# myrrix/myrrix-recommender

Measured on AMD Instinct MI355X. Metric: ALS rows solved/sec (full iteration) at k=64, higher is better.
Workload: dtype f32 storage; per-row Gramian: f16x2-split operands (22 bits), f32 accumulate; Cholesky f32

## Files before the change

### myrrix-recommender_amd/csrc/als_kernels.h

```cpp
#pragma once
#include <hip/hip_runtime.h>
#include <stdint.h>

#include <type_traits>

#include "work_plan.h"

namespace mals {

#ifndef MALS_WAVES
#define MALS_WAVES(T, MODE) ((T) <= 4 ? 4 : ((T) == 5 ? 3 : 2))
#endif
#ifndef MALS_WAVES_H
#define MALS_WAVES_H(T, MODE) ((T) <= 2 ? 5 : ((T) <= 4 ? 3 : 2))
#endif

typedef float f32x4 __attribute__((ext_vector_type(4)));
typedef double f64x4 __attribute__((ext_vector_type(4)));

__host__ __device__ constexpr int tri(int T) { return T * (T + 1) / 2; }
__host__ __device__ constexpr int tidx(int T, int i, int j) { return i * T - (i * (i - 1)) / 2 + (j - i); }

constexpr int GRAMIAN_FLUSH_BINADES = 5;
constexpr int YMAX_SLOTS = 64;
// ... 971 lines not shown
    } else {
#pragma unroll
      for (int t = 0; t < tri(T); ++t) acc[t] = f32x4{0.f, 0.f, 0.f, 0.f};
    }
    float bpart[T];
#pragma unroll
    for (int v = 0; v < T; ++v) bpart[v] = 0.f;
#ifdef MALS_PROFILING
    const int64_t trow = it / n_waves - p.trace_start;
    const bool tr = MODE == 0 && p.trace && wave < 64 && trow >= 0 && trow < 64;
    unsigned long long t0 = 0, t1 = 0, t2 = 0, t3 = 0;
    if (tr) t0 = __builtin_readcyclecounter();
    if (!(p.flags & 0x200)) gather_row<T, D, FULL>(p, cur.begin, cur.len, lane, pp, acc, bpart);
    if (tr) t1 = __builtin_readcyclecounter();
#else
    gather_row<T, D, FULL>(p, cur.begin, cur.len, lane, pp, acc, bpart);
#endif
    float bcol[T];
#pragma unroll
    for (int v = 0; v < T; ++v) bcol[v] = reduce_groups(bpart[v], lane);
    const bool prime_next = nxt.len > 0;
    if (prime_next) pp.ch = chunk_issue(p, nxt.begin, nxt.len, 0, lane);
    const WorkItem nxt2 = load_item(p, it + 2 * n_waves);
    if (MODE == 0) {
      const float wmax = p.refine_flag ? fmaxf(row_part_max<T>(acc, sG, lane), p.gramian_weight * __int_as_float(max_entry_bits<T>(acc, lane))) : 0.f;
      add_ridge<T, FULL>(p, acc, cur.len, lane);
      float minpiv = 3.0e38f;
      float xcol[T];
#ifdef MALS_PROFILING
      if (p.flags & 0x100) {
#pragma unroll
        for (int v = 0; v < T; ++v) xcol[v] = 1e-3f + 1e-9f * (bcol[v] + acc[tidx(T, v, v)][0] + acc[tidx(T, 0, v)][1]);
        if (prime_next) {
          chunk_weights(p, pp.ch);
          prime_row<T, D, FULL>(p, lane, pp);
        }
      } else
#endif
      {
        cholesky_tiles<T>(acc, lane, minpiv);
#ifdef MALS_PROFILING
        if (tr) t2 = __builtin_readcyclecounter();
#endif
        if (prime_next) {
          chunk_weights(p, pp.ch);
          prime_row<T, D, FULL>(p, lane, pp);
        }
        solve_tiles<T>(acc, bcol, xcol, lane);
      }
      store_row<T>(p, xcol, minpiv, wmax, cur.id, lane);
#ifdef MALS_PROFILING
      if (tr) {
        t3 = __builtin_readcyclecounter();
        if (lane == 0) {
          unsigned long long* o = p.trace + (trow * 64 + wave) * 6;
          o[0] = t0; o[1] = t1; o[2] = t2; o[3] = t3; o[4] = (unsigned long long)cur.len; o[5] = wall_clock64();
        }
      }
#endif
    } else {
      float* s = p.scratch + (int64_t)cur.id * ((tri(T) * 4 + T) * 64);
#pragma unroll
      for (int t = 0; t < tri(T); ++t) reinterpret_cast<f32x4*>(s)[t * 64 + lane] = acc[t];
#pragma unroll
      for (int v = 0; v < T; ++v) s[(tri(T) * 4 + v) * 64 + lane] = bcol[v];
      if (prime_next) {
        chunk_weights(p, pp.ch);
        prime_row<T, D, FULL>(p, lane, pp);
      }
    }
    if (nxt.len < 0) break;
    cur = nxt;
    nxt = nxt2;
    it += n_waves;
  }
}

template <int T, int MODE, bool FULL, int NTERM = 2>
__global__ __launch_bounds__(256, MALS_WAVES_H(T, MODE)) void als_persistent_kernel_h(SolveParams p) {
  __shared__ f32x4 sG[MODE == 0 ? tri(T) * 64 : 1];
  const int lane = threadIdx.x & 63;
  const int wave = uniform(blockIdx.x * 4 + (threadIdx.x >> 6));
  const int64_t n_waves = (int64_t)gridDim.x * 4;
  if (MODE == 0) {
    const f32x4* G4 = reinterpret_cast<const f32x4*>(p.Gf);
    for (int e = threadIdx.x; e < tri(T) * 64; e += 256) sG[e] = (p.flags & 2) ? f32x4{0.f, 0.f, 0.f, 0.f} : G4[e];
    __syncthreads();
  }
  int64_t it = wave;
  if (it >= p.n_work) return;
  if (p.zscale[2] == 0.f) return;
  const float zscale = __int_as_float(uniform(__float_as_int(p.zscale[0])));
  const float inv_s2 = __int_as_float(uniform(__float_as_int(p.zscale[1])));
  WorkItem cur = load_item(p, it);
  WorkItem nxt = load_item(p, it + n_waves);
  WorkItem nx2 = load_item(p, it + 2 * n_waves);
  constexpr int E = split_slots(T);
  float raw[T][E];
#pragma unroll
  for (int v = 0; v < T; ++v)
#pragma unroll
    for (int e = 0; e < E; ++e) raw[v][e] = 0.f;
  if (cur.len > 0) {
    Chunk ch = chunk_issue<true>(p, cur.begin, cur.len, 0, lane);
    Chunk nch = nxt.len > 0 ? chunk_issue<true>(p, nxt.begin, nxt.len, 0, lane) : ch;
    chunk_weights_h(p, ch, zscale);
    prime_row_h<T, E, FULL>(p, ch.col, lane, raw);
    for (;;) {
      const WorkItem nx3 = load_item(p, it + 3 * n_waves);
      f32x4 acc[tri(T)];
#pragma unroll
      for (int t = 0; t < tri(T); ++t) acc[t] = f32x4{0.f, 0.f, 0.f, 0.f};
      float bpart[T];
#pragma unroll
      for (int v = 0; v < T; ++v) bpart[v] = 0.f;
#ifdef MALS_PROFILING
      const int64_t trow = it / n_waves - p.trace_start;
      const bool tr = MODE == 0 && p.trace && wave < 64 && trow >= 0 && trow < 64;
      unsigned long long t0 = 0, t1 = 0, t2 = 0;
      if (tr) t0 = __builtin_readcyclecounter();
#endif
      gather_row_h<T, E, FULL, NTERM>(p, cur.begin, cur.len, lane, zscale, ch, nch.col, raw, acc, bpart);
#ifdef MALS_PROFILING
      if (tr) t1 = __builtin_readcyclecounter();
#endif
      float bcol[T];
#pragma unroll
      for (int v = 0; v < T; ++v) bcol[v] = reduce_groups(bpart[v], lane);
      ch = nch;
      if (nxt.len > 0) chunk_weights_h(p, ch, zscale);
      if (MODE == 0) {
        const float rmax = p.refine_flag ? __int_as_float(max_entry_bits<T>(acc, lane)) * inv_s2 : 0.f;
#pragma unroll
        for (int t = 0; t < tri(T); ++t) {
          const f32x4 g4 = sG[t * 64 + lane];
          if constexpr (T <= MALS_PK_MAXT) {
            acc[t] = __builtin_elementwise_fma(acc[t], f32x4{inv_s2, inv_s2, inv_s2, inv_s2}, g4);
          } else {
#pragma unroll
            for (int r = 0; r < 4; ++r) acc[t][r] = fmaf(acc[t][r], inv_s2, g4[r]);
          }
        }
        add_ridge<T, FULL>(p, acc, cur.len, lane);
        float minpiv = 3.0e38f, wmax;
        float xcol[T];
        if constexpr (T >= 2) {
          const float inv_s2row = row_scale<T>(acc, bcol, lane, wmax);
          cholesky_tiles<T, true>(acc, lane, minpiv);
          minpiv *= inv_s2row;
        } else {
          wmax = __int_as_float(max_entry_bits<T>(acc, lane));
          cholesky_tiles<T>(acc, lane, minpiv);
        }
#ifdef MALS_PROFILING
        if (tr) t2 = __builtin_readcyclecounter();
#endif
        solve_tiles<T>(acc, bcol, xcol, lane);
        store_row<T>(p, xcol, minpiv, fmaxf(rmax, p.gramian_weight * wmax), cur.id, lane);
#ifdef MALS_PROFILING
        if (tr) {
          const unsigned long long t3 = __builtin_readcyclecounter();
          if (lane == 0) {
            unsigned long long* o = p.trace + (trow * 64 + wave) * 6;
            o[0] = t0; o[1] = t1; o[2] = t2; o[3] = t3; o[4] = (unsigned long long)cur.len; o[5] = wall_clock64();
          }
        }
#endif
      } else {
        float* s = p.scratch + (int64_t)cur.id * ((tri(T) * 4 + T) * 64);
#pragma unroll
        for (int t = 0; t < tri(T); ++t) reinterpret_cast<f32x4*>(s)[t * 64 + lane] = acc[t] * inv_s2;
#pragma unroll
        for (int v = 0; v < T; ++v) s[(tri(T) * 4 + v) * 64 + lane] = bcol[v];
      }
      cur = nxt;
      nxt = nx2;
      nx2 = nx3;
      nch = nxt.len > 0 ? chunk_issue<true>(p, nxt.begin, nxt.len, 0, lane) : nch;
      it += n_waves;
      if (cur.len <= 0) break;
    }
  }
  if (MODE == 0) {
    while (cur.len == 0) {
      f32x4 acc[tri(T)];
#pragma unroll
      for (int t = 0; t < tri(T); ++t) acc[t] = sG[t * 64 + lane];
      float bcol[T];
#pragma unroll
      for (int v = 0; v < T; ++v) bcol[v] = 0.f;
      finish_row<T>(p, acc, bcol, 0, cur.id, lane);
      it += n_waves;
      cur = load_item(p, it);
    }
  }
}

template <int T>
__device__ __forceinline__ void add_slot(const float* __restrict__ s, int lane, f32x4 (&acc)[tri(T)], float (&bcol)[T]) {
  constexpr int PASSES = T >= 6 ? 2 : 1, PER = (tri(T) + PASSES - 1) / PASSES;
#pragma unroll
  for (int ps = 0; ps < PASSES; ++ps) {
    f32x4 part[PER];
#pragma unroll
    for (int t = 0; t < PER; ++t)
      if (ps * PER + t < tri(T)) part[t] = reinterpret_cast<const f32x4*>(s)[(ps * PER + t) * 64 + lane];
    if (ps == 0) {
      float bp[T];
#pragma unroll
      for (int v = 0; v < T; ++v) bp[v] = s[(tri(T) * 4 + v) * 64 + lane];
#pragma unroll
      for (int v = 0; v < T; ++v) bcol[v] += bp[v];
    }
#pragma unroll
    for (int t = 0; t < PER; ++t)
      if (ps * PER + t < tri(T)) acc[ps * PER + t] += part[t];
    if (PASSES > 1) __builtin_amdgcn_sched_barrier(0);
  }
}

template <int T>
__global__ __launch_bounds__(256) void als_prereduce_kernel(SolveParams p) {
  const int lane = threadIdx.x & 63;
  const int64_t wave = (int64_t)blockIdx.x * 4 + (threadIdx.x >> 6);
  if (wave >= p.n_work) return;
  RowC rc = p.rowsC[wave];
  rc.first_slot = uniform64(rc.first_slot);
  rc.nseg = uniform(rc.nseg);
  constexpr int SLOT = (tri(T) * 4 + T) * 64;
  float* s0 = p.scratch + rc.first_slot * (int64_t)SLOT;
  f32x4 acc[tri(T)];
  float bcol[T];
#pragma unroll
  for (int t = 0; t < tri(T); ++t) acc[t] = reinterpret_cast<const f32x4*>(s0)[t * 64 + lane];
#pragma unroll
  for (int v = 0; v < T; ++v) bcol[v] = s0[(tri(T) * 4 + v) * 64 + lane];
  for (int sgi = 1; sgi < rc.nseg; ++sgi) {
    add_slot<T>(s0 + sgi * (int64_t)SLOT, lane, acc, bcol);
  }
#pragma unroll
  for (int t = 0; t < tri(T); ++t) reinterpret_cast<f32x4*>(s0)[t * 64 + lane] = acc[t];
#pragma unroll
  for (int v = 0; v < T; ++v) s0[(tri(T) * 4 + v) * 64 + lane] = bcol[v];
}

template <int T, bool PERM = false>
__global__ __launch_bounds__(256, T >= 6 ? 2 : 1) void als_finish_kernel(SolveParams p) {
  const int lane = threadIdx.x & 63;
  const int64_t wave = (int64_t)blockIdx.x * 4 + (threadIdx.x >> 6);
  if (wave >= p.n_work) return;
  if (PERM && p.zscale[2] == 0.f) return;
  if (!PERM && (p.flags & 8) && p.zscale[2] != 0.f) return;
  RowC rc = p.rowsC[wave];
  rc.first_slot = uniform64(rc.first_slot);
  rc.row = uniform(rc.row);
  rc.nseg = uniform(rc.nseg);
// ... 792 lines not shown
```

### myrrix-recommender_amd/csrc/mals_api.hip

```cpp
#include "../../include/myrrix_als.h"
#include "als_kernels.h"
#include "dual_kernels.h"
#include "lds_kernels.h"
#include "host_eigen.h"
#include "host_solver.h"
#include "mals_internal.h"
#include "mals_handle.h"
#include "hip_buffer.h"
#include "work_plan.h"
#include "convergence.h"

#include <hip/hip_runtime.h>

#include <algorithm>
#include <chrono>
#include <cmath>
#include <cstdio>
#include <cstdlib>
#include <cstring>
#include <limits>
#include <memory>
#include <new>
#include <string>
#include <type_traits>
// ... 77 lines not shown
  HIPCHK(h, d_rows.alloc(rows.size()));
  HIPCHK(h, d_off.alloc(n_off));
  HIPCHK(h, d_unsorted.alloc(rows.size()));
  HIPCHK(h, hipMemcpyAsync(d_rows.get(), rows.data(), sizeof(BandRow) * rows.size(), hipMemcpyHostToDevice, h->stream));
  HIPCHK(h, hipMemsetAsync(d_unsorted.get(), 0, sizeof(int) * rows.size(), h->stream));
  hipLaunchKernelGGL(band_cuts_kernel, dim3((unsigned)rows.size(), BAND_CHECK_SLICES), dim3(256), 0, h->stream, s.col, d_rows.get(),
                     (int)bc.n_bands, bc.band_rows, d_off.get(), d_unsorted.get());
  HIPCHK(h, hipGetLastError());
  bc.off.resize(n_off);
  bc.unsorted.resize(rows.size());
  HIPCHK(h, hipMemcpyAsync(bc.off.data(), d_off.get(), sizeof(int64_t) * n_off, hipMemcpyDeviceToHost, h->stream));
  HIPCHK(h, hipMemcpyAsync(bc.unsorted.data(), d_unsorted.get(), sizeof(int) * rows.size(), hipMemcpyDeviceToHost, h->stream));
  HIPCHK(h, hipStreamSynchronize(h->stream));
  return MALS_OK;
}

int scan_shard(mals_handle h, SideState& s, BandCuts& bc) {
  s.max_abs_val = 0.f;
  s.mean_abs_val = 0.0;
  s.local_mean_abs_val = 0.0;
  if (s.nnz > 0) {
    HIPCHK(h, hipMemsetAsync(h->d_maxabs.get(), 0, 4 * sizeof(unsigned), h->stream));
    const unsigned blocks = (unsigned)std::min<int64_t>(4096, (s.nnz + 255) / 256);
    hipLaunchKernelGGL(max_abs_kernel, dim3(blocks), dim3(256), 0, h->stream, s.val, s.nnz, h->d_maxabs.get(),
                       reinterpret_cast<double*>(h->d_maxabs.get() + 2));
    HIPCHK(h, hipGetLastError());
    unsigned raw[4];
    HIPCHK(h, hipMemcpyAsync(raw, h->d_maxabs.get(), sizeof(raw), hipMemcpyDeviceToHost, h->stream));
    HIPCHK(h, hipStreamSynchronize(h->stream));
    std::memcpy(&s.max_abs_val, &raw[0], sizeof(float));
    double sum = 0.0;
    std::memcpy(&sum, &raw[2], sizeof(double));
    s.mean_abs_val = sum / (double)s.nnz;
    s.local_mean_abs_val = s.mean_abs_val;
  }
  s.local_max_abs_val = s.max_abs_val;
  s.col_min = 0;
  s.col_max = -1;
  if (s.nnz > 0) {
    const int init[2] = {std::numeric_limits<int>::max(), std::numeric_limits<int>::min()};
    HIPCHK(h, hipMemcpyAsync(h->d_colrange.get(), init, sizeof(init), hipMemcpyHostToDevice, h->stream));
    const unsigned blocks = (unsigned)std::min<int64_t>(4096, (s.nnz + 255) / 256);
    hipLaunchKernelGGL(col_range_kernel, dim3(blocks), dim3(256), 0, h->stream, s.col, s.nnz, h->d_colrange.get());
    HIPCHK(h, hipGetLastError());
    int range[2];
    HIPCHK(h, hipMemcpyAsync(range, h->d_colrange.get(), sizeof(range), hipMemcpyDeviceToHost, h->stream));
    HIPCHK(h, hipStreamSynchronize(h->stream));
    s.col_min = range[0];
    s.col_max = range[1];
    if (s.col_min < 0) return fail(h, MALS_INVALID_ARG, "negative column index");
  }
  if (int rc = find_band_cuts(h, s, bc)) return rc;
  {
    const char* e = std::getenv("MALS_BAND_FRONT");
    s.band_front = !e || std::atoi(e) != 0;
  }
  return MALS_OK;
}

int upload_work_lists(mals_handle h, SideState& s, const WorkPlan& plan, const BandCuts& bc) {
  s.chunks = plan.chunks;
  s.n_dual_rows = plan.n_dual_rows;
  if (std::getenv("MALS_DEBUG_LISTS")) {
    int64_t nd[4] = {0, 0, 0, 0}, ed[4] = {0, 0, 0, 0}, na = 0, nz = 0, n_long = 0;
    for (const ChunkRange& cr : s.chunks) {
      n_long += cr.nC;
      for (int c = 0; c < 4; ++c) {
        nd[c] += cr.nD[c];
        ed[c] += cr.nnzD[c];
      }
      na += cr.nA;
      nz += cr.nZ;
    }
    std::fprintf(stderr, "[lists] rows %lld: direct %lld (%lld entries), dual 1-16: %lld (%lld) 17-32: %lld (%lld) 33-48: %lld (%lld) 49-64: %lld (%lld), "
                         "zero-filled %lld, segments %lld of %lld long rows (%lld entries)\n",
                 (long long)s.n_local, (long long)na, (long long)plan.nnzA, (long long)nd[0], (long long)ed[0], (long long)nd[1], (long long)ed[1], (long long)nd[2],
                 (long long)ed[2], (long long)nd[3], (long long)ed[3], (long long)nz, (long long)plan.itemsB.size(), (long long)n_long, (long long)plan.nnzB);
    int64_t e_band = 0;
    for (const ChunkRange& cr : s.chunks) e_band += cr.nnzBand;
    std::fprintf(stderr, "[lists] bands %lld of %lld table rows (at least %lld entries per band): %lld banded rows (%lld entries) in %lld segments, "
                         "%lld long enough but unsorted\n",
                 (long long)bc.n_bands, (long long)bc.band_rows, (long long)bc.min_avg, (long long)plan.n_banded_rows, (long long)e_band,
                 (long long)plan.n_banded_segs, (long long)plan.n_unsorted);
  }
  if (!plan.itemsA.empty()) {
    HIPCHK(h, s.itemsA.alloc(plan.itemsA.size()));
    HIPCHK(h, hipMemcpy(s.itemsA.get(), plan.itemsA.data(), sizeof(WorkItem) * plan.itemsA.size(), hipMemcpyHostToDevice));
  }
  if (!plan.itemsB.empty()) {
    HIPCHK(h, s.itemsB.alloc(plan.itemsB.size()));
    HIPCHK(h, hipMemcpy(s.itemsB.get(), plan.itemsB.data(), sizeof(WorkItem) * plan.itemsB.size(), hipMemcpyHostToDevice));
    HIPCHK(h, s.rowsC.alloc(plan.rowsC.size()));
    HIPCHK(h, hipMemcpy(s.rowsC.get(), plan.rowsC.data(), sizeof(RowC) * plan.rowsC.size(), hipMemcpyHostToDevice));
    HIPCHK(h, s.scratch.alloc((size_t)(plan.n_slots * slot_floats(h->T))));
  }
  return MALS_OK;
}

int64_t wanted_chunk_rows(mals_handle h, const SideState& s) { return s.chunk_rows_override >= 0 ? s.chunk_rows_override : h->cfg.chunk_rows; }

int build_work_lists(mals_handle h, SideState& s) {
  BandCuts bc;
  WorkPlan plan;
  s.n_dual_rows = 0;
  if (int rc = scan_shard(h, s, bc)) return rc;
  if (const char* why = plan_work_lists(s.h_row_ptr.data(), s.n_local, h->cfg.segment_nnz, wanted_chunk_rows(h, s), h->dual_blocks, h->n_cu, bc, plan))
    return fail(h, MALS_INVALID_ARG, why);
  return upload_work_lists(h, s, plan, bc);
}

int validate_matrix(mals_handle h, int side) {
  SideState& s = h->side[side];
  if (s.h_row_ptr.size() != (size_t)s.n_local + 1 || s.h_row_ptr[0] != 0 || s.h_row_ptr[(size_t)s.n_local] != s.nnz)
    return fail(h, MALS_INVALID_ARG, "row_ptr must have n_rows_local+1 entries, start at 0 and end at nnz");
  return MALS_OK;
}

int validate_columns(mals_handle h, int side) {
  const SideState& s = h->side[side];
  const SideState& o = h->side[1 - side];
  if (s.nnz > 0 && o.n_total > 0 && (int64_t)s.col_max >= o.n_total)
    return fail(h, MALS_INVALID_ARG, "column index outside the opposite side's factor replica");
  return MALS_OK;
}

int begin_timed(mals_handle h, int kind, double bytes, PendingEvent& pe) {
  pe.kind = kind;
  pe.bytes = bytes;
  if (!h->timing) return MALS_OK;
  HIPCHK(h, pe.ev.ensure());
  HIPCHK(h, hipEventRecord(pe.ev.begin, h->stream));
  return MALS_OK;
}
int end_timed(mals_handle h, PendingEvent& pe) {
  if (!h->timing) return MALS_OK;
  HIPCHK(h, hipEventRecord(pe.ev.end, h->stream));
  h->pending.push_back(std::move(pe));
  return MALS_OK;
}
int drain_events(mals_handle h) {
  const std::vector<PendingEvent> pending = std::move(h->pending);
  h->pending.clear();
  for (const PendingEvent& pe : pending) {
    HIPCHK(h, hipEventSynchronize(pe.ev.end));
    float ms = 0.f;
    HIPCHK(h, hipEventElapsedTime(&ms, pe.ev.begin, pe.ev.end));
    mals_stats& st = h->stats;
    switch (pe.kind) {
      case 0: st.rows_ms += ms; st.rows_launches += 1; st.rows_bytes += pe.bytes; break;
      case 1: st.segments_ms += ms; st.segments_launches += 1; st.segments_bytes += pe.bytes; break;
      case 2: st.finish_ms += ms; st.finish_launches += 1; st.finish_bytes += pe.bytes; break;
      case 4: st.dual_ms += ms; st.dual_launches += 1; st.dual_bytes += pe.bytes; break;
      case 5: st.rotate_ms += ms; st.rotate_launches += 1; st.rotate_bytes += pe.bytes; break;
      default: st.gramian_ms += ms; st.gramian_launches += 1; st.gramian_bytes += pe.bytes; break;
    }
  }
  return MALS_OK;
}

template <int MIN_T = 1, typename F>
int dispatch_T(mals_handle h, F&& f) {
  if (h->T == MIN_T) return f(std::integral_constant<int, MIN_T>());
  if constexpr (MIN_T < 8) return dispatch_T<MIN_T + 1>(h, f);
  return fail(h, MALS_INVALID_ARG, "unsupported feature count");
}
constexpr int gather_depth(int T) { return T <= 3 ? 4 : T == 4 ? MALS_D4 : 2; }

constexpr int64_t GRAMIAN_SPLIT_MIN_ROWS = 262144;
inline int64_t gramian_slab_rows(int64_t n_rows) {
  static const int64_t forced = std::getenv("MALS_GRAMIAN_SLAB_ROWS") ? std::atoll(std::getenv("MALS_GRAMIAN_SLAB_ROWS")) : 0;
  if (forced > 0) return forced;
  int64_t slab = 512;
  while (slab < 2048 && n_rows / (2 * slab) / 4 >= 1024) slab *= 2;
  return slab;
}

template <int T>
int launch_gramian_T(mals_handle h, SideState& s, const float* M, int64_t n_rows, double* G_out, float* Gf_out, unsigned* ymax) {
  const int k = h->cfg.features;
  const int elems = tri(T) * 256;
  static const bool force_f64 = std::getenv("MALS_GRAMIAN_F64") != nullptr;
  if (n_rows >= GRAMIAN_SPLIT_MIN_ROWS && !force_f64) {
    const int64_t slab_rows = gramian_slab_rows(n_rows);
    int64_t n_slabs = (n_rows + slab_rows - 1) / slab_rows;
    n_slabs = (n_slabs + 3) & ~(int64_t)3;
    constexpr int GROUPS = 64;
    const size_t slab_bytes = sizeof(float) * (size_t)n_slabs * tri(T) * 256;
    const size_t bytes = 2 * slab_bytes + sizeof(double) * (size_t)GROUPS * tri(T) * 256 + sizeof(int) * (size_t)n_slabs;
    if (s.partials.capacity() < bytes) HIPCHK(h, s.partials.alloc(bytes));
// ... 21 lines not shown
  if (ymax) HIPCHK(h, hipMemsetAsync(ymax, 0x7f, sizeof(unsigned), h->stream));
  hipLaunchKernelGGL((gramian_partial_kernel<T>), dim3((unsigned)(n_waves / 4)), dim3(256), 0, h->stream, M, n_rows, k,
                     rows_per_wave, partials);
  hipLaunchKernelGGL((gramian_finalize_kernel<T, true, 16>), dim3(elems / 16), dim3(256), 0, h->stream, partials, n_waves,
                     k, G_out, Gf_out);
  HIPCHK(h, hipGetLastError());
  return MALS_OK;
}

int launch_gramian(mals_handle h, SideState& s, const float* M, int64_t n_rows, double* G_out, float* Gf_out, unsigned* ymax = nullptr) {
  return dispatch_T(h, [&](auto t) { return launch_gramian_T<t()>(h, s, M, n_rows, G_out, Gf_out, ymax); });
}

template <typename K>
int persistent_grid(mals_handle h, K kernel, int64_t n_work, unsigned* grid, bool front = false, int block = 256, int resident_per_cu = 0) {
  const int64_t groups = (n_work + block / 64 - 1) / (block / 64);
  if (front) {
    *grid = (unsigned)std::max<int64_t>(1, groups);
    return MALS_OK;
  }
  int per_cu = resident_per_cu;
  if (!per_cu) HIPCHK(h, hipOccupancyMaxActiveBlocksPerMultiprocessor(&per_cu, kernel, 256, 0));
  if (per_cu < 1) per_cu = 1;
  per_cu *= 16;
  if (const char* e = std::getenv("MALS_BLOCKS_PER_CU")) per_cu = std::max(1, std::atoi(e)) * (256 / block);
  const int64_t cap = (int64_t)h->n_cu * per_cu;
  *grid = (unsigned)std::max<int64_t>(1, std::min<int64_t>(groups, cap));
  return MALS_OK;
}

enum { LISTS_ROWS = 1, LISTS_DUAL_ROWS = 2, LISTS_LONG = 4 };

template <typename KR, typename KS, typename KRF, typename KSF, typename KC, typename KCF, typename KP>
struct ListKernels {
  KR rows;
  KS segments;
  KRF rows_f32;
  KSF segments_f32;
  KC finish;
  KCF finish_f32;
  KP prereduce;
  int block;
  int resident_per_cu;
};
template <typename KR, typename KS, typename KRF, typename KSF, typename KC, typename KCF, typename KP>
ListKernels(KR, KS, KRF, KSF, KC, KCF, KP, int, int) -> ListKernels<KR, KS, KRF, KSF, KC, KCF, KP>;

template <typename K, typename KF>
int launch_persistent(mals_handle h, K kernel, KF fallback, int block, int resident_per_cu, const SolveParams& p, int kind, double bytes, bool front) {
  PendingEvent pe;
  unsigned grid = 1;
  if (int rc = persistent_grid(h, kernel, p.n_work, &grid, front, block, resident_per_cu)) return rc;
  if (int rc = begin_timed(h, kind, bytes, pe)) return rc;
  hipLaunchKernelGGL(kernel, dim3(grid), dim3(block), 0, h->stream, p);
  if constexpr (!std::is_same<KF, std::nullptr_t>::value) {
    SolveParams pf = p;
    pf.flags |= 8;
    if (int rc = persistent_grid(h, fallback, p.n_work, &grid)) return rc;
    grid = std::min<unsigned>(grid, (unsigned)h->n_cu * 8u);
    hipLaunchKernelGGL(fallback, dim3(grid), dim3(256), 0, h->stream, pf);
  }
  return end_timed(h, pe);
}

template <typename LK>
int launch_lists(mals_handle h, SideState& s, SolveParams p, int chunk, int which, const LK& fam) {
  const double per = 4.0 * p.k + 8.0;
  const ChunkRange& cr = s.chunks[(size_t)chunk];
  const bool own = which & LISTS_ROWS, longs = which & LISTS_LONG, dual_rows_too = which & LISTS_DUAL_ROWS;
  const WorkItem *A = s.itemsA.get() + cr.offA, *B = s.itemsB.get() + cr.offB;
  const int64_t n_plain = cr.nB - cr.nBand, n_dual = cr.n_dual();
  struct Run {
    const WorkItem* items;
    int64_t n;
    double bytes;
    int kind;
    bool front;
  };
  const Run runs[4] = {
      {B, longs ? n_plain : 0, (double)(cr.nnzB - cr.nnzBand) * per, 1, false},
      {B + n_plain, longs ? cr.nBand : 0, (double)cr.nnzBand * per, 1, s.band_front},
      {A, own ? cr.nA : 0, (double)cr.nnzA * per + (double)cr.nA * per, 0, false},
      {A + cr.nA, dual_rows_too ? n_dual : 0, (double)cr.nnz_dual() * per + (double)n_dual * per, 0, false}};
  for (const Run& r : runs) {
    if (!r.n) continue;
    p.n_work = r.n;
    p.items = r.items;
    if (int rc = r.kind ? launch_persistent(h, fam.segments, fam.segments_f32, fam.block, fam.resident_per_cu, p, 1, r.bytes, r.front)
                        : launch_persistent(h, fam.rows, fam.rows_f32, fam.block, fam.resident_per_cu, p, 0, r.bytes, r.front))
      return rc;
  }
  if (longs && cr.nC) {
    PendingEvent pe;
    if (int rc = begin_timed(h, 2, (double)cr.nC * per, pe)) return rc;
    if (cr.nP) {
      p.n_work = cr.nP;
      p.rowsC = s.rowsC.get() + cr.offP;
      hipLaunchKernelGGL(fam.prereduce, dim3((unsigned)((cr.nP + 3) / 4)), dim3(256), 0, h->stream, p);
    }
    p.n_work = cr.nC;
    p.rowsC = s.rowsC.get() + cr.offC;
    hipLaunchKernelGGL(fam.finish, dim3((unsigned)((cr.nC + 3) / 4)), dim3(256), 0, h->stream, p);
    if constexpr (!std::is_same<decltype(fam.finish_f32), std::nullptr_t>::value) {
      SolveParams pf = p;
      pf.flags |= 8;
      hipLaunchKernelGGL(fam.finish_f32, dim3((unsigned)((cr.nC + 3) / 4)), dim3(256), 0, h->stream, pf);
    }
    if (int rc = end_timed(h, pe)) return rc;
  }
  if (own && cr.nZ) {
    hipLaunchKernelGGL(zero_rows_kernel, dim3((unsigned)((cr.nZ + 31) / 32)), dim3(256), 0, h->stream,
                       A + cr.nA + n_dual, cr.nZ, p.k, p.out);
  }
  HIPCHK(h, hipGetLastError());
  return MALS_OK;
}

template <int T, bool FULL>
int launch_solve_TF(mals_handle h, SideState& s, const SolveParams& p, int chunk, int which) {
  constexpr int D = gather_depth(T);
  constexpr auto rows_f32 = als_persistent_kernel<T, D, 0, FULL>;
  constexpr auto segments_f32 = als_persistent_kernel<T, D, 1, FULL>;
  if constexpr (T == 8 && FULL) {
    if (h->split_f16 && h->lds_gather && p.Gperm)
      return launch_lists(h, s, p, chunk, which, ListKernels{als_lds_kernel_h<0>, als_lds_kernel_h<1>, rows_f32, segments_f32, als_finish_kernel<T, true>,
                                                             als_finish_kernel<T, false>, als_prereduce_kernel<T>, 64, 8});
  }
  if constexpr (T == 4) {
    if (h->split3)
      return launch_lists(h, s, p, chunk, which, ListKernels{als_persistent_kernel_h<T, 0, FULL, 3>, als_persistent_kernel_h<T, 1, FULL, 3>, rows_f32,
                                                             segments_f32, als_finish_kernel<T>, nullptr, als_prereduce_kernel<T>, 256, 0});
  }
  if (h->split_f16)
    return launch_lists(h, s, p, chunk, which, ListKernels{als_persistent_kernel_h<T, 0, FULL>, als_persistent_kernel_h<T, 1, FULL>, rows_f32,
                                                           segments_f32, als_finish_kernel<T>, nullptr, als_prereduce_kernel<T>, 256, 0});
  return launch_lists(h, s, p, chunk, which,
                      ListKernels{rows_f32, segments_f32, nullptr, nullptr, als_finish_kernel<T>, nullptr, als_prereduce_kernel<T>, 256, 0});
}

int launch_solve(mals_handle h, SideState& s, const SolveParams& p, int chunk, int which) {
  return dispatch_T(h, [&](auto t) {
    return p.k == 16 * t() ? launch_solve_TF<t(), true>(h, s, p, chunk, which) : launch_solve_TF<t(), false>(h, s, p, chunk, which);
  });
}

int launch_refine(mals_handle h, const RefineParams& q) {
  const int64_t rows = q.row_end - q.row_begin;
  const unsigned grid = (unsigned)std::max<int64_t>(1, std::min<int64_t>((rows + 255) / 256, (int64_t)h->n_cu * 8));
  return dispatch_T(h, [&](auto t) -> int {
    hipLaunchKernelGGL((als_refine_kernel<t()>), dim3(grid), dim3(256), 0, h->stream, q);
    HIPCHK(h, hipGetLastError());
    return MALS_OK;
  });
}

int launch_gramian_ref(mals_handle h, const SideState& o) {
  const unsigned grid = (unsigned)std::max<int64_t>(1, std::min<int64_t>((o.n_total + 63) / 64, (int64_t)h->n_cu * 2));
  return dispatch_T(h, [&](auto t) -> int {
    hipLaunchKernelGGL(gramian_ref_latch_kernel, dim3(1), dim3(1), 0, h->stream, h->d_gref_state.get());
    hipLaunchKernelGGL((gramian_ref_kernel<t()>), dim3(grid), dim3(256), 0, h->stream, o.F, o.n_total, h->cfg.features, h->d_gref_state.get(),
                       h->d_gref_part.get(), h->d_Gref.get());
    HIPCHK(h, hipGetLastError());
    return MALS_OK;
  });
}

int launch_exact(mals_handle h, const RefineParams& q, int level) {
  const int k = h->cfg.features;
  const size_t lds = sizeof(double) * ((size_t)k * (k + 1) + 2 * (size_t)k) + sizeof(float) * (size_t)k + sizeof(int) * 256;
  if (!h->exact_ready) {
// ... 376 lines not shown
  std::unique_ptr<mals_handle_s> owner(new (std::nothrow) mals_handle_s());
  const mals_handle h = owner.get();
  if (!h) return create_fail(MALS_OOM, "mals_create: out of host memory");
  h->cfg = *cfg;
  h->cfg.flags &= 3;
#ifdef MALS_PROFILING
  if (const char* dbg = std::getenv("MALS_DEBUG_FLAGS")) h->cfg.flags |= (std::atoi(dbg) & 0xff) << 8;
#endif
  if (h->cfg.segment_nnz <= 0) h->cfg.segment_nnz = 4096;
  if (h->cfg.chunk_rows < 0) h->cfg.chunk_rows = 0;
  h->cfg.segment_nnz = (h->cfg.segment_nnz + 3) & ~3;
  h->T = (cfg->features + 15) / 16;
  switch (cfg->gramian_mode) {
    case MALS_GRAMIAN_AUTO: h->split_f16 = h->T >= 2; break;
    case MALS_GRAMIAN_FP32: h->split_f16 = false; break;
    case MALS_GRAMIAN_SPLIT_F16: h->split_f16 = true; break;
    case MALS_GRAMIAN_SPLIT3_F16:
      if (h->T != 4) return create_fail(MALS_INVALID_ARG, "mals_create: MALS_GRAMIAN_SPLIT3_F16 is built for 49..64 features");
      h->split_f16 = h->split3 = true;
      break;
    default: return create_fail(MALS_INVALID_ARG, "mals_create: unknown gramian_mode");
  }
  if (cfg->alpha < 0.0) h->split_f16 = false;
  switch (cfg->solve_mode) {
    case MALS_SOLVE_AUTO: h->dual_blocks = h->T >= 3 ? dual_max_blocks(h->T) : 0; break;
    case MALS_SOLVE_DIRECT: h->dual_blocks = 0; break;
    case MALS_SOLVE_DUAL: h->dual_blocks = dual_max_blocks(h->T); break;
    default: return create_fail(MALS_INVALID_ARG, "mals_create: unknown solve_mode");
  }
  if (h->cfg.flags != 0 || !(cfg->alpha > 0.0)) h->dual_blocks = 0;
  {
    hipDeviceProp_t prop;
    if (hipGetDeviceProperties(&prop, cfg->device) == hipSuccess && prop.multiProcessorCount > 0)
      h->n_cu = prop.multiProcessorCount;
  }
  std::memset(&h->stats, 0, sizeof(h->stats));
  h->stats.struct_size = (int32_t)sizeof(mals_stats);
  hipError_t st = hipSetDevice(cfg->device);
  if (st == hipSuccess) st = h->d_bad.alloc(4);
  if (st == hipSuccess) st = h->h_bad.alloc(4);
  if (st == hipSuccess) st = h->d_zscale.alloc(4);
  if (st == hipSuccess) st = h->d_maxabs.alloc(4);
  if (st == hipSuccess) st = h->d_colrange.alloc(2);
  if (st == hipSuccess) st = h->d_refined.alloc(1);
  if (st == hipSuccess) st = h->d_gref_state.alloc(4);
  if (st == hipSuccess) st = hipMemset(h->d_gref_state.get(), 0, 4 * sizeof(int));
  if (st == hipSuccess) st = hipMemset(h->d_refined.get(), 0, sizeof(unsigned long long));
  if (st == hipSuccess) st = hipMemset(h->d_zscale.get(), 0, 4 * sizeof(float));
  if (st == hipSuccess) st = hipMemset(h->d_bad.get(), 0xff, 4 * sizeof(unsigned long long));
  if (st != hipSuccess) return create_fail(MALS_HIP_ERROR, "mals_create: device " + std::to_string(cfg->device) + ": " + hipGetErrorString(st));
  if (const char* e = std::getenv("MALS_REFINE_LIMIT")) h->refine_limit = std::max(0.f, (float)std::atof(e));
  if (h->ev_ready.ensure(hipEventDisableTiming) != hipSuccess || h->ev_refine.ensure(hipEventDisableTiming) != hipSuccess)
    return create_fail(MALS_HIP_ERROR, "mals_create: creating the handle's events failed");
  h->lds_gather = h->cfg.features == 128;
  if (const char* e = std::getenv("MALS_LDS_GATHER")) h->lds_gather = h->lds_gather && std::atoi(e) != 0;
  if (const char* e = std::getenv("MALS_OVERLAP")) h->overlap = std::atoi(e) != 0;
  if (h->overlap) {
    bool ok = h->ev_fork.ensure(hipEventDisableTiming) == hipSuccess;
    for (int i = 0; i < 2 && ok; ++i) ok = h->aux[i].ensure() == hipSuccess && h->ev_join[i].ensure(hipEventDisableTiming) == hipSuccess;
    if (!ok) h->overlap = false;
  }
#ifdef MALS_PROFILING
  if (std::getenv("MALS_DEBUG_TRACE")) {
    (void)h->d_trace.alloc(64 * 64 * 6);
    (void)hipMemset(h->d_trace.get(), 0, 64 * 64 * 6 * sizeof(unsigned long long));
  }
#endif
  t_create_error.clear();
  malsi_serving_create(h);
  *out = owner.release();
  return MALS_OK;
}

int mals_destroy(mals_handle h) {
  if (!h) return MALS_INVALID_ARG;
  (void)hipSetDevice(h->cfg.device);
  malsi_serving_stop_front(h);
  (void)hipStreamSynchronize(h->stream);
  for (const Stream& a : h->aux)
    if (a) (void)hipStreamSynchronize(a);
  if (h->d_trace) {
    std::vector<unsigned long long> t(64 * 64 * 6);
    (void)hipMemcpy(t.data(), h->d_trace.get(), t.size() * sizeof(unsigned long long), hipMemcpyDeviceToHost);
    for (int r = 0; r < 64; r += 21)
      for (int w = 0; w < 4; w += 1) {
        const unsigned long long* o = &t[(size_t)(r * 64 + w) * 6];
        std::fprintf(stderr, "[trace] iter %2d wave %2d len %5llu gather %7llu chol %7llu solve+store %7llu gap_to_prev_end %lld\n", r, w, o[4],
                     o[1] - o[0], o[2] - o[1], o[3] - o[2], r ? (long long)(o[0] - t[(size_t)((r - 1) * 64 + w) * 6 + 3]) : 0ll);
      }
    for (int w = 0; w < 4; ++w) {
      const unsigned long long* a = &t[(size_t)w * 6];
      const unsigned long long* b = &t[(size_t)(63 * 64 + w) * 6];
      if (b[5] > a[5]) std::fprintf(stderr, "[trace] wave %d: %llu cycles in %llu wall ticks (100 MHz) = %.0f MHz; %.0f cycles per row\n", w, b[3] - a[3], b[5] - a[5], 100.0 * (double)(b[3] - a[3]) / (double)(b[5] - a[5]), (double)(b[3] - a[3]) / 63.0);
    }
  }
  malsi_serving_free(h);
  delete h;
  return MALS_OK;
}

int mals_features(mals_handle h) { return h ? h->cfg.features : 0; }

const char* mals_last_error(mals_handle h) { return h ? h->err.c_str() : "null handle"; }

int mals_set_stream(mals_handle h, void* hip_stream) {
  if (!h) return MALS_INVALID_ARG;
  h->stream = (hipStream_t)hip_stream;
  return MALS_OK;
}

int mals_set_factor_rows(mals_handle h, int side, int64_t n_rows_total) {
  CHECK_SIDE(h, side);
  if (n_rows_total <= 0) return fail(h, MALS_INVALID_ARG, "n_rows_total must be positive");
  if (int rc = use_device(h)) return rc;
  SideState& s = h->side[side];
  s.F = nullptr;
  const size_t n = (size_t)n_rows_total * (size_t)h->cfg.features;
  HIPCHK(h, s.F_own.alloc(n));
  s.F = s.F_own.get();
  HIPCHK(h, hipMemsetAsync(s.F, 0, sizeof(float) * n, h->stream));
  s.n_total = n_rows_total;
  s.G_valid = false;
  ++s.F_epoch;
  if (side == MALS_SIDE_X) h->grown_users_end.store(-1);
  malsi_generation_drop_recent(h, side);
  if (side == MALS_SIDE_X) popular_touch(h, false);
  if (side == MALS_SIDE_Y) h->lsh.clear();
  return MALS_OK;
}

int mals_bind_factors(mals_handle h, int side, float* device_ptr, int64_t n_rows_total) {
  CHECK_SIDE(h, side);
  if (!device_ptr || n_rows_total <= 0) return fail(h, MALS_INVALID_ARG, "null buffer or non-positive row count");
  if (int rc = use_device(h)) return rc;
  SideState& s = h->side[side];
  s.F_own.reset();
  s.F = device_ptr;
  s.n_total = n_rows_total;
  s.G_valid = false;
  ++s.F_epoch;
  if (side == MALS_SIDE_X) h->grown_users_end.store(-1);
  malsi_generation_drop_recent(h, side);
  if (side == MALS_SIDE_X) popular_touch(h, false);
  if (side == MALS_SIDE_Y) h->lsh.clear();
  return MALS_OK;
}

int mals_factor_device_ptr(mals_handle h, int side, void** out_device_ptr, int64_t* out_n_rows_total) {
  CHECK_SIDE(h, side);
  if (out_device_ptr) *out_device_ptr = h->side[side].F;
  if (out_n_rows_total) *out_n_rows_total = h->side[side].n_total;
  return h->side[side].F ? MALS_OK : fail(h, MALS_INVALID_ARG, "factor replica not allocated");
}

int mals_set_matrix(mals_handle h, int side, int64_t row_offset, int64_t n_rows_local, int64_t nnz, const int64_t* row_ptr,
                    const int32_t* col_idx, const float* val, int mem_kind) {
  CHECK_SIDE(h, side);
  if (row_offset < 0 || n_rows_local < 0 || nnz < 0 || !row_ptr || (nnz > 0 && (!col_idx || !val)))
    return fail(h, MALS_INVALID_ARG, "bad matrix arguments");
  if (n_rows_local > std::numeric_limits<int32_t>::max())
    return fail(h, MALS_INVALID_ARG, "at most 2^31-1 local rows per handle");
  if (int rc = use_device(h)) return rc;
  SideState& s = h->side[side];
  HIPCHK(h, hipStreamSynchronize(h->stream));
  free_matrix(s);
  if (side == MALS_SIDE_X) malsi_clear_known_items(h);
  if (side == MALS_SIDE_X) malsi_popular_new_generation(h, true);
// ... 929 lines not shown
```

### myrrix-recommender_amd/csrc/work_plan.h

```cpp
#pragma once

#include "band_plan.h"

#include <algorithm>
#include <cstdint>
#include <limits>
#include <utility>
#include <vector>

namespace mals {

struct WorkItem {
  int64_t begin;
  int32_t len;
  int32_t id;
};
struct RowC {
  int64_t first_slot;
  int32_t row;
  int32_t nseg;
  int32_t stride;
  int32_t pad_;
};
constexpr int FINISH_GROUP = 32;

struct BandCuts {
  int64_t n_bands = 1, band_rows = 0, min_avg = 0;
  std::vector<int64_t> row;
  std::vector<int64_t> off;
  std::vector<int> unsorted;
};

struct ChunkRange {
  int64_t row0 = 0, row1 = 0;
  int64_t offA = 0, nA = 0, nnzA = 0, offB = 0, nB = 0, nnzB = 0, offC = 0, nC = 0;
  int64_t offP = 0, nP = 0;
  int64_t nD[4] = {0, 0, 0, 0}, nnzD[4] = {0, 0, 0, 0}, nZ = 0;
  int64_t nBand = 0, nnzBand = 0;
  int64_t n_dual() const { return nD[0] + nD[1] + nD[2] + nD[3]; }
  int64_t nnz_dual() const { return nnzD[0] + nnzD[1] + nnzD[2] + nnzD[3]; }
};

struct WorkPlan {
  std::vector<WorkItem> itemsA;
  std::vector<WorkItem> itemsB;
  std::vector<RowC> rowsC;
  std::vector<ChunkRange> chunks;
  int64_t n_slots = 0;
  int64_t nnzA = 0, nnzB = 0;
  int64_t n_dual_rows = 0;
  int64_t n_banded_rows = 0, n_banded_segs = 0, n_unsorted = 0;
};

inline int64_t plan_chunk_rows(int64_t chunk_rows, int64_t n_local) { return chunk_rows > 0 ? chunk_rows : std::max<int64_t>(n_local, 1); }

inline const char* plan_work_lists(const int64_t* rp, int64_t n, int seg, int64_t chunk_rows_wanted, int dual_blocks, int n_cu,
                                   const BandCuts& bc, WorkPlan& plan) {
  plan = WorkPlan();
  const int64_t chunk_rows = plan_chunk_rows(chunk_rows_wanted, n);
  const int n_chunks = (int)std::max<int64_t>(1, (n + chunk_rows - 1) / chunk_rows);
  std::vector<WorkItem>& order = plan.itemsA;
  std::vector<WorkItem>& segs = plan.itemsB;
  std::vector<RowC>& rowsC = plan.rowsC;
  std::vector<std::pair<int32_t, WorkItem>> band_segs;
  std::vector<BandPiece> pieces;
  std::vector<RowC> groups;
  size_t bc_next = 0;
  order.reserve((size_t)n);
  int64_t& slot = plan.n_slots;
  plan.chunks.assign((size_t)n_chunks, ChunkRange());
  std::vector<int64_t> count((size_t)seg + 2);
  for (int c = 0; c < n_chunks; ++c) {
    ChunkRange& cr = plan.chunks[(size_t)c];
    const int64_t r0 = cr.row0 = std::min(n, c * chunk_rows), r1 = cr.row1 = std::min(n, (c + 1) * chunk_rows);
    cr.offA = (int64_t)order.size();
    cr.offB = (int64_t)segs.size();
    cr.offC = (int64_t)rowsC.size();
    std::fill(count.begin(), count.end(), 0);
    const int64_t dual_len = 16 * (int64_t)dual_blocks;
    int64_t n_short = 0, n_direct = 0, n_empty = 0;
    for (int64_t r = r0; r < r1; ++r) {
      const int64_t len = rp[r + 1] - rp[r];
      if (len < 0) return "row_ptr must be non-decreasing";
      if (len <= seg) {
        ++count[(size_t)(seg - len)];
        ++n_short;
        if (len == 0) {
          ++n_empty;
        } else if (len <= dual_len) {
          const int cls = (int)((len - 1) >> 4);
          ++cr.nD[cls];
          cr.nnzD[cls] += len;
        } else {
          ++n_direct;
          cr.nnzA += len;
        }
      } else {
        cr.nnzB += len;
      }
    }
    int64_t seg_b = seg;
    {
      const int64_t want_segments = (int64_t)n_cu * 4;
      const int64_t lo = std::min<int64_t>(512, seg);
      seg_b = std::max<int64_t>(lo, std::min<int64_t>(seg, (cr.nnzB + want_segments - 1) / want_segments));
      seg_b = (seg_b + 31) & ~(int64_t)31;
      if (seg_b > seg) seg_b = seg;
    }
    int64_t acc = cr.offA;
    for (size_t b = 0; b < count.size(); ++b) {
      const int64_t cnt = count[b];
      count[b] = acc;
      acc += cnt;
    }
    order.resize((size_t)(cr.offA + n_short));
    for (int64_t r = r0; r < r1; ++r) {
      const int64_t len = rp[r + 1] - rp[r];
      if (len <= seg) {
        WorkItem& w = order[(size_t)count[(size_t)(seg - len)]++];
        w.begin = rp[r];
        w.len = (int32_t)len;
        w.id = (int32_t)r;
      } else {
        const int64_t nseg = (len + seg_b - 1) / seg_b;
        int64_t per = (len + nseg - 1) / nseg;
        per = (per + 3) & ~(int64_t)3;
        RowC rc;
        rc.first_slot = slot;
        rc.row = (int32_t)r;
        rc.nseg = 0;
        rc.stride = 1;
        rc.pad_ = 0;
        pieces.clear();
        if (bc_next < bc.row.size() && bc.row[bc_next] == r) {
          if (bc.unsorted[bc_next]) ++plan.n_unsorted;
          else if (!band_plan_row(&bc.off[bc_next * (size_t)(bc.n_bands + 1)], bc.n_bands, len, seg, pieces)) pieces.clear();
          ++bc_next;
        }
        if (!pieces.empty()) {
          ++plan.n_banded_rows;
          plan.n_banded_segs += (int64_t)pieces.size();
          cr.nnzBand += len;
          for (const BandPiece& pc : pieces) {
            if (slot >= std::numeric_limits<int32_t>::max()) return "too many row segments";
            WorkItem sg;
            sg.begin = rp[r] + pc.begin;
            sg.len = pc.len;
            sg.id = (int32_t)slot++;
            band_segs.emplace_back(pc.band, sg);
            ++rc.nseg;
          }
        } else {
          for (int64_t b = 0; b < len; b += per) {
            if (slot >= std::numeric_limits<int32_t>::max()) return "too many row segments";
            WorkItem sg;
            sg.begin = rp[r] + b;
            sg.len = (int32_t)std::min(per, len - b);
            sg.id = (int32_t)slot++;
            segs.push_back(sg);
            ++rc.nseg;
          }
        }
        if (rc.nseg > FINISH_GROUP) {
          const int32_t grp_len = FINISH_GROUP;
          for (int32_t g0 = 0; g0 < rc.nseg; g0 += grp_len) {
            RowC grp;
            grp.first_slot = rc.first_slot + g0;
            grp.row = (int32_t)r;
            grp.nseg = std::min<int32_t>(grp_len, rc.nseg - g0);
            grp.stride = 1;
            grp.pad_ = 0;
            groups.push_back(grp);
          }
          rc.nseg = (rc.nseg + grp_len - 1) / grp_len;
          rc.stride = grp_len;
        }
        rowsC.push_back(rc);
      }
    }
    const int64_t n_dual = cr.n_dual();
    if (n_empty > 0 && n_dual > 0) {
      auto first = order.begin() + (size_t)(cr.offA + n_direct);
      std::rotate(first, first + (size_t)n_dual, first + (size_t)n_dual + 1);
    }
    cr.nA = n_direct + (n_empty > 0 ? 1 : 0);
    cr.nZ = n_empty > 0 ? n_empty - 1 : 0;
    plan.n_dual_rows += n_dual;
    cr.nBand = (int64_t)band_segs.size();
    cr.nB = (int64_t)segs.size() - cr.offB + cr.nBand;
    cr.nC = (int64_t)rowsC.size() - cr.offC;
    cr.offP = (int64_t)rowsC.size();
    cr.nP = (int64_t)groups.size();
    rowsC.insert(rowsC.end(), groups.begin(), groups.end());
    groups.clear();
    std::stable_sort(segs.begin() + cr.offB, segs.end(), [](const WorkItem& a, const WorkItem& b) { return a.len > b.len; });
    std::stable_sort(band_segs.begin(), band_segs.end(), [](const std::pair<int32_t, WorkItem>& a, const std::pair<int32_t, WorkItem>& b) {
      return a.first != b.first ? a.first < b.first : a.second.len > b.second.len;
    });
    for (const std::pair<int32_t, WorkItem>& bs : band_segs) segs.push_back(bs.second);
    band_segs.clear();
    plan.nnzA += cr.nnzA;
    plan.nnzB += cr.nnzB;
  }
  return nullptr;
}

}
```

Before: 138.7 million.

## Merge consecutive long-row segments into capped runs to cut partial-slot overhead

Long rows split into segments now have adjacent segments (same band) merged into longer work items, capped by a per-launch entry budget derived from wave count and segment size. This reduces the number of partial Gramian slots written to scratch and later reduced, cutting per-item fixed overhead such as the scratch store and finish work. It risks load imbalance when merged items become long relative to the launch. Profiling hooks for segment launches and extra plan statistics are also added under debug flags.

```diff
diff --git a/myrrix-recommender_amd/csrc/als_kernels.h b/myrrix-recommender_amd/csrc/als_kernels.h
--- a/myrrix-recommender_amd/csrc/als_kernels.h
+++ b/myrrix-recommender_amd/csrc/als_kernels.h
@@ -1077,6 +1077,9 @@
   const int lane = threadIdx.x & 63;
   const int wave = uniform(blockIdx.x * 4 + (threadIdx.x >> 6));
   const int64_t n_waves = (int64_t)gridDim.x * 4;
+#ifdef MALS_PROFILING
+  const unsigned long long t_entry = __builtin_readcyclecounter();
+#endif
   if (MODE == 0) {
     const f32x4* G4 = reinterpret_cast<const f32x4*>(p.Gf);
     for (int e = threadIdx.x; e < tri(T) * 64; e += 256) sG[e] = (p.flags & 2) ? f32x4{0.f, 0.f, 0.f, 0.f} : G4[e];
@@ -1101,6 +1104,9 @@
     Chunk nch = nxt.len > 0 ? chunk_issue<true>(p, nxt.begin, nxt.len, 0, lane) : ch;
     chunk_weights_h(p, ch, zscale);
     prime_row_h<T, E, FULL>(p, ch.col, lane, raw);
+#ifdef MALS_PROFILING
+    unsigned long long t_item = t_entry;
+#endif
     for (;;) {
       const WorkItem nx3 = load_item(p, it + 3 * n_waves);
       f32x4 acc[tri(T)];
@@ -1113,11 +1119,13 @@
       const int64_t trow = it / n_waves - p.trace_start;
       const bool tr = MODE == 0 && p.trace && wave < 64 && trow >= 0 && trow < 64;
       unsigned long long t0 = 0, t1 = 0, t2 = 0;
-      if (tr) t0 = __builtin_readcyclecounter();
+      const int64_t every = p.trace_start > 0 ? p.trace_start : 1;
+      const bool tr1 = MODE == 1 && p.trace && it % every == 0 && it / every < 64 * 64;
+      if (tr || tr1) t0 = __builtin_readcyclecounter();
 #endif
       gather_row_h<T, E, FULL, NTERM>(p, cur.begin, cur.len, lane, zscale, ch, nch.col, raw, acc, bpart);
 #ifdef MALS_PROFILING
-      if (tr) t1 = __builtin_readcyclecounter();
+      if (tr || tr1) t1 = __builtin_readcyclecounter();
 #endif
       float bcol[T];
 #pragma unroll
@@ -1167,6 +1175,14 @@
         for (int t = 0; t < tri(T); ++t) reinterpret_cast<f32x4*>(s)[t * 64 + lane] = acc[t] * inv_s2;
 #pragma unroll
         for (int v = 0; v < T; ++v) s[(tri(T) * 4 + v) * 64 + lane] = bcol[v];
+#ifdef MALS_PROFILING
+        const unsigned long long t3 = __builtin_readcyclecounter();
+        if (tr1 && lane == 0) {
+          unsigned long long* o = p.trace + (it / every) * 6;
+          o[0] = t_item; o[1] = t0; o[2] = t1; o[3] = t3; o[4] = (unsigned long long)cur.len; o[5] = wall_clock64();
+        }
+        t_item = t3;
+#endif
       }
       cur = nxt;
       nxt = nx2;
diff --git a/myrrix-recommender_amd/csrc/mals_api.hip b/myrrix-recommender_amd/csrc/mals_api.hip
--- a/myrrix-recommender_amd/csrc/mals_api.hip
+++ b/myrrix-recommender_amd/csrc/mals_api.hip
@@ -183,6 +183,15 @@
                          "%lld long enough but unsorted\n",
                  (long long)bc.n_bands, (long long)bc.band_rows, (long long)bc.min_avg, (long long)plan.n_banded_rows, (long long)e_band,
                  (long long)plan.n_banded_segs, (long long)plan.n_unsorted);
+    int64_t n_plain = 0, n_band = 0, n_groups = 0;
+    for (const ChunkRange& cr : s.chunks) {
+      n_plain += cr.nB - cr.nBand;
+      n_band += cr.nBand;
+      n_groups += cr.nP;
+    }
+    std::fprintf(stderr, "[lists] runs: %lld segments in %lld items of list B (%lld plain, %lld banded), a partial slot of %lld bytes each; %lld slot groups\n",
+                 (long long)plan.n_segments, (long long)plan.n_slots, (long long)n_plain, (long long)n_band, (long long)(slot_floats(h->T) * 4),
+                 (long long)n_groups);
   }
   if (!plan.itemsA.empty()) {
     HIPCHK(h, s.itemsA.alloc(plan.itemsA.size()));
@@ -200,12 +209,23 @@
 
 int64_t wanted_chunk_rows(mals_handle h, const SideState& s) { return s.chunk_rows_override >= 0 ? s.chunk_rows_override : h->cfg.chunk_rows; }
 
+RunRule run_rule(mals_handle h) {
+  RunRule rule;
+  if (h->T > 4) return rule;
+  const int per_simd = h->split_f16 ? MALS_WAVES_H(h->T, 1) : MALS_WAVES(h->T, 1);
+  rule.waves = (int64_t)h->n_cu * 4 * per_simd;
+  rule.longest = 3 * (int64_t)h->cfg.segment_nnz / 2;
+  if (const char* e = std::getenv("MALS_RUN_ENTRIES")) rule.max_entries = std::max<int64_t>(0, std::atoll(e));
+  return rule;
+}
+
 int build_work_lists(mals_handle h, SideState& s) {
   BandCuts bc;
   WorkPlan plan;
   s.n_dual_rows = 0;
   if (int rc = scan_shard(h, s, bc)) return rc;
-  if (const char* why = plan_work_lists(s.h_row_ptr.data(), s.n_local, h->cfg.segment_nnz, wanted_chunk_rows(h, s), h->dual_blocks, h->n_cu, bc, plan))
+  if (const char* why = plan_work_lists(s.h_row_ptr.data(), s.n_local, h->cfg.segment_nnz, wanted_chunk_rows(h, s), h->dual_blocks, h->n_cu, bc, plan,
+                                        run_rule(h)))
     return fail(h, MALS_INVALID_ARG, why);
   return upload_work_lists(h, s, plan, bc);
 }
@@ -393,10 +413,18 @@
       {B + n_plain, longs ? cr.nBand : 0, (double)cr.nnzBand * per, 1, s.band_front},
       {A, own ? cr.nA : 0, (double)cr.nnzA * per + (double)cr.nA * per, 0, false},
       {A + cr.nA, dual_rows_too ? n_dual : 0, (double)cr.nnz_dual() * per + (double)n_dual * per, 0, false}};
+#ifdef MALS_PROFILING
+  unsigned long long* const trace = p.trace;
+  const char* tl = std::getenv("MALS_DEBUG_TRACE_LAUNCH");
+  const int traced_launch = tl ? std::atoi(tl) : 2;
+#endif
   for (const Run& r : runs) {
     if (!r.n) continue;
     p.n_work = r.n;
     p.items = r.items;
+#ifdef MALS_PROFILING
+    p.trace = &r - runs == traced_launch ? trace : nullptr;
+#endif
     if (int rc = r.kind ? launch_persistent(h, fam.segments, fam.segments_f32, fam.block, fam.resident_per_cu, p, 1, r.bytes, r.front)
                         : launch_persistent(h, fam.rows, fam.rows_f32, fam.block, fam.resident_per_cu, p, 0, r.bytes, r.front))
       return rc;
@@ -939,7 +967,27 @@
   if (h->d_trace) {
     std::vector<unsigned long long> t(64 * 64 * 6);
     (void)hipMemcpy(t.data(), h->d_trace.get(), t.size() * sizeof(unsigned long long), hipMemcpyDeviceToHost);
-    for (int r = 0; r < 64; r += 21)
+    const char* tl = std::getenv("MALS_DEBUG_TRACE_LAUNCH");
+    if (tl && std::atoi(tl) < 2) {
+      unsigned long long n = 0, len = 0, total = 0, gather = 0, head = 0, tail = 0;
+      for (size_t i = 0; i < 64 * 64; ++i) {
+        const unsigned long long* o = &t[i * 6];
+        if (!o[3]) continue;
+        ++n;
+        len += o[4];
+        total += o[3] - o[0];
+        gather += o[2] - o[1];
+        head += o[1] - o[0];
+        tail += o[3] - o[2];
+      }
+      if (n)
+        std::fprintf(stderr, "[trace] segments launch %d: %llu sampled items, mean %.0f entries, %.0f cycles per item: gather %.0f, before it %.0f, after it %.0f "
+                             "(%.1f %% outside the gather)\n",
+                     std::atoi(tl), n, (double)len / n, (double)total / n, (double)gather / n, (double)head / n, (double)tail / n,
+                     100.0 * (double)(total - gather) / (double)total);
+      std::fill(t.begin(), t.end(), 0ull);
+    }
+    for (int r = 0; r < 64 && t[3]; r += 21)
       for (int w = 0; w < 4; w += 1) {
         const unsigned long long* o = &t[(size_t)(r * 64 + w) * 6];
         std::fprintf(stderr, "[trace] iter %2d wave %2d len %5llu gather %7llu chol %7llu solve+store %7llu gap_to_prev_end %lld\n", r, w, o[4],
diff --git a/myrrix-recommender_amd/csrc/work_plan.h b/myrrix-recommender_amd/csrc/work_plan.h
--- a/myrrix-recommender_amd/csrc/work_plan.h
+++ b/myrrix-recommender_amd/csrc/work_plan.h
@@ -23,6 +23,23 @@
   int32_t pad_;
 };
 constexpr int FINISH_GROUP = 32;
+
+struct RunRule {
+  int64_t waves = 0;
+  int64_t longest = 0;
+  int64_t max_entries = -1;
+  int64_t cap(int64_t launch_entries) const {
+    int64_t c = max_entries >= 0 ? max_entries : waves > 0 ? launch_entries / (4 * waves) : 0;
+    if (max_entries < 0 && longest > 0 && c > longest) c = longest;
+    return c < (int64_t(1) << 30) ? c : (int64_t(1) << 30);
+  }
+};
+
+inline void plan_runs(int64_t n, int64_t seg_len, int64_t cap, std::vector<int32_t>& per_run) {
+  const int64_t most = std::max<int64_t>(1, seg_len > 0 ? cap / seg_len : 1);
+  const int64_t n_runs = (n + most - 1) / most;
+  for (int64_t i = 0; i < n_runs; ++i) per_run.push_back((int32_t)(n / n_runs + (i < n % n_runs ? 1 : 0)));
+}
 
 struct BandCuts {
   int64_t n_bands = 1, band_rows = 0, min_avg = 0;
@@ -47,6 +64,7 @@
   std::vector<RowC> rowsC;
   std::vector<ChunkRange> chunks;
   int64_t n_slots = 0;
+  int64_t n_segments = 0;
   int64_t nnzA = 0, nnzB = 0;
   int64_t n_dual_rows = 0;
   int64_t n_banded_rows = 0, n_banded_segs = 0, n_unsorted = 0;
@@ -55,7 +73,7 @@
 inline int64_t plan_chunk_rows(int64_t chunk_rows, int64_t n_local) { return chunk_rows > 0 ? chunk_rows : std::max<int64_t>(n_local, 1); }
 
 inline const char* plan_work_lists(const int64_t* rp, int64_t n, int seg, int64_t chunk_rows_wanted, int dual_blocks, int n_cu,
-                                   const BandCuts& bc, WorkPlan& plan) {
+                                   const BandCuts& bc, WorkPlan& plan, const RunRule& runs = RunRule()) {
   plan = WorkPlan();
   const int64_t chunk_rows = plan_chunk_rows(chunk_rows_wanted, n);
   const int n_chunks = (int)std::max<int64_t>(1, (n + chunk_rows - 1) / chunk_rows);
@@ -64,8 +82,19 @@
   std::vector<RowC>& rowsC = plan.rowsC;
   std::vector<std::pair<int32_t, WorkItem>> band_segs;
   std::vector<BandPiece> pieces;
+  std::vector<int32_t> per_run;
   std::vector<RowC> groups;
   size_t bc_next = 0;
+  auto banded_pieces = [&](int64_t r, int64_t len, size_t& cursor) {
+    bool unsorted = false;
+    pieces.clear();
+    if (cursor < bc.row.size() && bc.row[cursor] == r) {
+      if (bc.unsorted[cursor]) unsorted = true;
+      else if (!band_plan_row(&bc.off[cursor * (size_t)(bc.n_bands + 1)], bc.n_bands, len, seg, pieces)) pieces.clear();
+      ++cursor;
+    }
+    return unsorted;
+  };
   order.reserve((size_t)n);
   int64_t& slot = plan.n_slots;
   plan.chunks.assign((size_t)n_chunks, ChunkRange());
@@ -78,7 +107,9 @@
     cr.offC = (int64_t)rowsC.size();
     std::fill(count.begin(), count.end(), 0);
     const int64_t dual_len = 16 * (int64_t)dual_blocks;
-    int64_t n_short = 0, n_direct = 0, n_empty = 0;
+    int64_t n_short = 0, n_direct = 0, n_empty = 0, nnz_band = 0;
+    const bool cap_from_launch = runs.max_entries < 0 && runs.waves > 0;
+    size_t bc_scan = bc_next;
     for (int64_t r = r0; r < r1; ++r) {
       const int64_t len = rp[r + 1] - rp[r];
       if (len < 0) return "row_ptr must be non-decreasing";
@@ -97,8 +128,13 @@
         }
       } else {
         cr.nnzB += len;
+        if (cap_from_launch) {
+          banded_pieces(r, len, bc_scan);
+          if (!pieces.empty()) nnz_band += len;
+        }
       }
     }
+    const int64_t cap_plain = runs.cap(cr.nnzB - nnz_band), cap_band = runs.cap(nnz_band);
     int64_t seg_b = seg;
     {
       const int64_t want_segments = (int64_t)n_cu * 4;
@@ -131,34 +167,32 @@
         rc.nseg = 0;
         rc.stride = 1;
         rc.pad_ = 0;
-        pieces.clear();
-        if (bc_next < bc.row.size() && bc.row[bc_next] == r) {
-          if (bc.unsorted[bc_next]) ++plan.n_unsorted;
-          else if (!band_plan_row(&bc.off[bc_next * (size_t)(bc.n_bands + 1)], bc.n_bands, len, seg, pieces)) pieces.clear();
-          ++bc_next;
-        }
-        if (!pieces.empty()) {
+        if (banded_pieces(r, len, bc_next)) ++plan.n_unsorted;
+        const bool banded = !pieces.empty();
+        if (banded) {
           ++plan.n_banded_rows;
           plan.n_banded_segs += (int64_t)pieces.size();
           cr.nnzBand += len;
-          for (const BandPiece& pc : pieces) {
+        } else {
+          for (int64_t b = 0; b < len; b += per) pieces.push_back(BandPiece{b, (int32_t)std::min(per, len - b), 0});
+        }
+        plan.n_segments += (int64_t)pieces.size();
+        for (size_t i0 = 0; i0 < pieces.size();) {
+          size_t i1 = i0 + 1;
+          while (i1 < pieces.size() && pieces[i1].band == pieces[i0].band) ++i1;
+          per_run.clear();
+          plan_runs((int64_t)(i1 - i0), pieces[i0].len, banded ? cap_band : cap_plain, per_run);
+          for (const int32_t in_run : per_run) {
             if (slot >= std::numeric_limits<int32_t>::max()) return "too many row segments";
             WorkItem sg;
-            sg.begin = rp[r] + pc.begin;
-            sg.len = pc.len;
+            sg.begin = rp[r] + pieces[i0].begin;
+            sg.len = 0;
+            for (int32_t j = 0; j < in_run; ++j) sg.len += pieces[i0 + (size_t)j].len;
             sg.id = (int32_t)slot++;
-            band_segs.emplace_back(pc.band, sg);
+            if (banded) band_segs.emplace_back(pieces[i0].band, sg);
+            else segs.push_back(sg);
             ++rc.nseg;
-          }
-        } else {
-          for (int64_t b = 0; b < len; b += per) {
-            if (slot >= std::numeric_limits<int32_t>::max()) return "too many row segments";
-            WorkItem sg;
-            sg.begin = rp[r] + b;
-            sg.len = (int32_t)std::min(per, len - b);
-            sg.id = (int32_t)slot++;
-            segs.push_back(sg);
-            ++rc.nseg;
+            i0 += (size_t)in_run;
           }
         }
         if (rc.nseg > FINISH_GROUP) {
```

Result: no change. 138.7 million (-0.0%).
